# jc-bao/gym-xarm

Measured on AMD Instinct MI355X. Metric: env steps/sec (whole node), XarmPDPickAndPlace-v0, higher is better.
Workload: dtype f32

## Files before the change

### gym_xarm_amd/csrc/xarm_dev.h

```cpp
#pragma once
#include <hip/hip_runtime.h>
#include <stdio.h>
#include <stdlib.h>
#include <string.h>
#include <new>
#include "../../include/xarm_hip.h"
#include "xarm_core.h"
#include "xarm_reach_core.h"
#include "xarm_handover_core.h"
#include "xarm_handover2_core.h"
#include "xarm_stack_core.h"
#include "xarm_rearrange_core.h"
#include "xarm_coop_core.h"
#include "xarm_handover_coop_core.h"
#include "xarm_reach_coop_core.h"

namespace xd {

constexpr int WG = 64;

struct DevLds {
    float *base;
    __device__ __forceinline__ float &operator[](int i) const { return base[i * WG]; }
};

struct KParams {
    float *state;
    int64_t stride;
    int64_t num_envs;
    xk::EnvCfg cfg;
    int auto_reset;
    int state_dim;
    int coop_limit;
    int eject_coop_cap;
    xr::EnvCfg rcfg;
    xh::EnvCfg hcfg;
};

__device__ __forceinline__ int64_t late_index(int64_t e) {
    int lo = (int)e, hi = (int)(e >> 32);
    asm volatile("" : "+v"(lo), "+v"(hi) : : "memory");
    return ((int64_t)hi << 32) | (uint32_t)lo;
}

__device__ __forceinline__ void load_state(const KParams &P, int64_t e, xk::EnvState<float> &s) {
    const float *S = P.state + e;
    const int64_t n = P.stride;
#pragma unroll
    for (int i = 0; i < 9; i++) { s.q[i] = S[(xk::S_Q + i) * n]; s.qd[i] = S[(xk::S_QD + i) * n]; }
#pragma unroll
    for (int i = 0; i < 3; i++) {
        s.bp[i] = S[(xk::S_BP + i) * n]; s.bv[i] = S[(xk::S_BV + i) * n];
        s.bw[i] = S[(xk::S_BW + i) * n]; s.goal[i] = S[(xk::S_GOAL + i) * n];
    }
#pragma unroll
    for (int i = 0; i < 4; i++) s.bq[i] = S[(xk::S_BQ + i) * n];
#pragma unroll
    for (int i = 0; i < 8; i++) { s.lam_t[i] = S[(xk::S_LT + i) * n]; s.lam_p[i] = S[(xk::S_LP + i) * n]; }
    s.touch = S[xk::S_TOUCH * n]; s.mug = S[xk::S_MUG * n]; s.steps = S[xk::S_STEPS * n]; s.episode = S[xk::S_EPISODE * n];
}

__device__ __forceinline__ void store_state(const KParams &P, int64_t e, const xk::EnvState<float> &s) {
    float *S = P.state + e;
    const int64_t n = P.stride;
#pragma unroll
    for (int i = 0; i < 9; i++) { S[(xk::S_Q + i) * n] = s.q[i]; S[(xk::S_QD + i) * n] = s.qd[i]; }
#pragma unroll
    for (int i = 0; i < 3; i++) {
        S[(xk::S_BP + i) * n] = s.bp[i]; S[(xk::S_BV + i) * n] = s.bv[i];
        S[(xk::S_BW + i) * n] = s.bw[i]; S[(xk::S_GOAL + i) * n] = s.goal[i];
    }
#pragma unroll
    for (int i = 0; i < 4; i++) S[(xk::S_BQ + i) * n] = s.bq[i];
#pragma unroll
    for (int i = 0; i < 8; i++) { S[(xk::S_LT + i) * n] = s.lam_t[i]; S[(xk::S_LP + i) * n] = s.lam_p[i]; }
    S[xk::S_TOUCH * n] = s.touch; S[xk::S_MUG * n] = s.mug; S[xk::S_STEPS * n] = s.steps; S[xk::S_EPISODE * n] = s.episode;
}

__device__ __forceinline__ void write_obs(const float (&obs)[xk::OBS_DIM], const xk::EnvState<float> &s, int64_t e,
                                          float *obs_out, float *ag_out, float *dg_out) {
    float4 *o = reinterpret_cast<float4 *>(obs_out + e * xk::OBS_DIM);
#pragma unroll
    for (int k = 0; k < xk::OBS_DIM / 4; k++) o[k] = make_float4(obs[4 * k], obs[4 * k + 1], obs[4 * k + 2], obs[4 * k + 3]);
#pragma unroll
    for (int k = 0; k < 3; k++) { ag_out[e * 3 + k] = s.bp[k]; dg_out[e * 3 + k] = s.goal[k]; }
}

constexpr int FAST_LDS_FLOATS = xk::LDS_FLOATS - xk::LDS_TBL;

struct FastLds {
    float *base;
    __device__ __forceinline__ float &operator[](int i) const { return base[(i - xk::LDS_TBL) * WG]; }
};

constexpr int COOP_ENVS = WG / xc::GL;
constexpr int HO_COOP_LDS_FLOATS = xk::LDS_T;

__device__ __forceinline__ int64_t xcd_contiguous_block() {
    const unsigned b = blockIdx.x, nwg = gridDim.x, xcd = b & 7u, q = nwg >> 3, r = nwg & 7u;
    return (int64_t)((xcd < r ? xcd * (q + 1) : r * (q + 1) + (xcd - r) * q) + (b >> 3));
}

struct DppXchg {
    __device__ __forceinline__ float from0(float v) const { return __int_as_float(__builtin_amdgcn_update_dpp(0, __float_as_int(v), 0xA0, 0xF, 0xF, true)); }
    __device__ __forceinline__ float from1(float v) const { return __int_as_float(__builtin_amdgcn_update_dpp(0, __float_as_int(v), 0xF5, 0xF, 0xF, true)); }
    __device__ __forceinline__ float partner(float v) const { return __int_as_float(__builtin_amdgcn_update_dpp(0, __float_as_int(v), 0xB1, 0xF, 0xF, true)); }
};

struct HoStage {
    int tick0, tick1;
    float *qt;
    uint8_t *flag;
};
__device__ __forceinline__ void ho_load_qt(const KParams &P, const HoStage &S, int64_t e, int arm, float (&qt)[9]) {
#pragma unroll
    for (int i = 0; i < 9; i++) qt[i] = S.qt[(9 * arm + i) * P.stride + e];
}
__device__ __forceinline__ void ho_store_qt(const KParams &P, const HoStage &S, int64_t e, int arm, const float (&qt)[9]) {
#pragma unroll
    for (int i = 0; i < 9; i++) S.qt[(9 * arm + i) * P.stride + e] = qt[i];
}
__device__ __forceinline__ void ho_load(const KParams &P, int64_t e, int arm, xh::Lane<float> &L) {
    const float *S = P.state + e;
    const int64_t n = P.stride;
#pragma unroll
    for (int i = 0; i < 9; i++) { L.st.q[i] = S[(xh::H_Q + 9 * arm + i) * n]; L.st.qd[i] = S[(xh::H_QD + 9 * arm + i) * n]; }
    L.ft = S[(xh::H_FT + arm) * n];
#pragma unroll
    for (int i = 0; i < 3; i++) {
        L.st.bp[i] = S[(xh::H_BP + i) * n]; L.st.bv[i] = S[(xh::H_BV + i) * n];
        L.st.bw[i] = S[(xh::H_BW + i) * n]; L.st.goal[i] = S[(xh::H_GOAL + i) * n];
    }
#pragma unroll
    for (int i = 0; i < 4; i++) { L.st.bq[i] = S[(xh::H_BQ + i) * n]; L.st.lam_p[i] = S[(xh::H_LP + 4 * arm + i) * n]; L.st.lam_p[4 + i] = 0.f; }
#pragma unroll
    for (int i = 0; i < 8; i++) L.st.lam_t[i] = S[(xh::H_LT + i) * n];
    L.st.touch = S[(xh::H_TOUCH + arm) * n]; L.st.mug = S[(xh::H_MUG + arm) * n];
    L.st.steps = S[xh::H_STEPS * n]; L.st.episode = S[xh::H_EPISODE * n];
}

__device__ __forceinline__ void ho_store(const KParams &P, int64_t e, int arm, const xh::Lane<float> &L) {
    float *S = P.state + e;
    const int64_t n = P.stride;
#pragma unroll
    for (int i = 0; i < 9; i++) { S[(xh::H_Q + 9 * arm + i) * n] = L.st.q[i]; S[(xh::H_QD + 9 * arm + i) * n] = L.st.qd[i]; }
    S[(xh::H_FT + arm) * n] = L.ft;
#pragma unroll
    for (int i = 0; i < 4; i++) S[(xh::H_LP + 4 * arm + i) * n] = L.st.lam_p[i];
    S[(xh::H_TOUCH + arm) * n] = L.st.touch; S[(xh::H_MUG + arm) * n] = L.st.mug;
    if (arm == 0) {
#pragma unroll
        for (int i = 0; i < 3; i++) {
            S[(xh::H_BP + i) * n] = L.st.bp[i]; S[(xh::H_BV + i) * n] = L.st.bv[i];
            S[(xh::H_BW + i) * n] = L.st.bw[i]; S[(xh::H_GOAL + i) * n] = L.st.goal[i];
        }
#pragma unroll
        for (int i = 0; i < 4; i++) S[(xh::H_BQ + i) * n] = L.st.bq[i];
#pragma unroll
        for (int i = 0; i < 8; i++) S[(xh::H_LT + i) * n] = L.st.lam_t[i];
        S[xh::H_STEPS * n] = L.st.steps; S[xh::H_EPISODE * n] = L.st.episode;
    }
}

__device__ __forceinline__ void ho_write_obs(const xh::Lane<float> &L, int64_t e, int arm, float *obs_out, float *ag_out, float *dg_out) {
    float o8[8];
    xh::arm_obs(L, arm, o8);
    float *o = obs_out + e * xh::OBS_DIM;
#pragma unroll
    for (int k = 0; k < 8; k++) o[13 + 8 * arm + k] = o8[k];
    if (arm == 0) {
#pragma unroll
        for (int k = 0; k < 3; k++) { o[k] = L.st.bp[k]; o[7 + k] = L.st.bv[k]; o[10 + k] = L.st.bw[k]; ag_out[e * 3 + k] = L.st.bp[k]; dg_out[e * 3 + k] = L.st.goal[k]; }
#pragma unroll
        for (int k = 0; k < 4; k++) o[3 + k] = L.st.bq[k];
    }
}

__global__ __launch_bounds__(WG) void k_init(KParams P);
__global__ __launch_bounds__(WG) void k_step(KParams P, const float *__restrict__ actions, float *__restrict__ obs_out,
                                             float *__restrict__ ag_out, float *__restrict__ dg_out,
                                             float *__restrict__ rew_out, uint8_t *__restrict__ done_out,
                                             uint8_t *__restrict__ succ_out, float *__restrict__ term_obs,
                                             int *__restrict__ done_list, int *__restrict__ done_count,
                                             const int *__restrict__ list, const int *__restrict__ count);
__global__ __launch_bounds__(WG) void k_step_fast(KParams P, const float *__restrict__ actions, float *__restrict__ obs_out,
                                                  float *__restrict__ ag_out, float *__restrict__ dg_out,
                                                  float *__restrict__ rew_out, uint8_t *__restrict__ done_out,
                                                  uint8_t *__restrict__ succ_out, float *__restrict__ term_obs,
                                                  int *__restrict__ done_list, int *__restrict__ done_count,
                                                  int *__restrict__ eject_list, int *__restrict__ eject_count);
__global__ __launch_bounds__(WG) void k_step_lazy(KParams P, const float *__restrict__ actions, float *__restrict__ obs_out,
                                                  float *__restrict__ ag_out, float *__restrict__ dg_out,
                                                  float *__restrict__ rew_out, uint8_t *__restrict__ done_out,
                                                  uint8_t *__restrict__ succ_out);
__global__ __launch_bounds__(WG) void k_reset(KParams P, const int *__restrict__ list, const int *__restrict__ count,
                                              float *__restrict__ obs_out, float *__restrict__ ag_out,
                                              float *__restrict__ dg_out);
__global__ __launch_bounds__(WG) void k_reset_coop(KParams P, const int *__restrict__ list, const int *__restrict__ count,
                                                   float *__restrict__ obs_out, float *__restrict__ ag_out,
                                                   float *__restrict__ dg_out);
__global__ __launch_bounds__(WG) void k_step_coop(KParams P, const float *__restrict__ actions, float *__restrict__ obs_out,
                                                  float *__restrict__ ag_out, float *__restrict__ dg_out,
                                                  float *__restrict__ rew_out, uint8_t *__restrict__ done_out,
                                                  uint8_t *__restrict__ succ_out, float *__restrict__ term_obs,
                                                  int *__restrict__ done_list, int *__restrict__ done_count);
__global__ __launch_bounds__(WG) void k_step_coop_list(KParams P, const float *__restrict__ actions, float *__restrict__ obs_out,
                                                       float *__restrict__ ag_out, float *__restrict__ dg_out,
                                                       float *__restrict__ rew_out, uint8_t *__restrict__ done_out,
                                                       uint8_t *__restrict__ succ_out, float *__restrict__ term_obs,
                                                       int *__restrict__ done_list, int *__restrict__ done_count,
                                                       const int *__restrict__ list, const int *__restrict__ count);
__global__ __launch_bounds__(WG) void k_step_fast_stage(KParams P, const float *__restrict__ actions, float *__restrict__ obs_out,
                                                        float *__restrict__ ag_out, float *__restrict__ dg_out,
                                                        float *__restrict__ rew_out, uint8_t *__restrict__ done_out,
                                                        uint8_t *__restrict__ succ_out, float *__restrict__ term_obs,
                                                        int *__restrict__ done_list, int *__restrict__ done_count,
                                                        int *__restrict__ eject_list, int *__restrict__ eject_count, HoStage stage);
__global__ __launch_bounds__(WG) void k_step_from_stage(KParams P, const float *__restrict__ actions, float *__restrict__ obs_out,
                                                        float *__restrict__ ag_out, float *__restrict__ dg_out,
                                                        float *__restrict__ rew_out, uint8_t *__restrict__ done_out,
                                                        uint8_t *__restrict__ succ_out, float *__restrict__ term_obs,
                                                        int *__restrict__ done_list, int *__restrict__ done_count,
                                                        const int *__restrict__ list, const int *__restrict__ count, HoStage stage);
__global__ __launch_bounds__(WG) void k_step_coop_list_stage(KParams P, const float *__restrict__ actions, float *__restrict__ obs_out,
                                                             float *__restrict__ ag_out, float *__restrict__ dg_out,
                                                             float *__restrict__ rew_out, uint8_t *__restrict__ done_out,
                                                             uint8_t *__restrict__ succ_out, float *__restrict__ term_obs,
                                                             int *__restrict__ done_list, int *__restrict__ done_count,
                                                             const int *__restrict__ list, const int *__restrict__ count, HoStage stage);
__global__ __launch_bounds__(WG) void k_substeps(KParams P, const float *__restrict__ qt_in, int n);
__global__ void k_compact_mask(const uint8_t *__restrict__ mask, int64_t n, int *__restrict__ list, int *__restrict__ count);
__global__ void k_get_state(KParams P, float *__restrict__ out);
__global__ void k_set_state(KParams P, const float *__restrict__ in);
__global__ void k_compute_reward(int reward_type, const float *__restrict__ ag, const float *__restrict__ g, int64_t n,
                                 float *__restrict__ out);
__global__ __launch_bounds__(WG) void k_reach_init(KParams P);
__global__ __launch_bounds__(WG) void k_reach_step(KParams P, const float *__restrict__ actions, float *__restrict__ obs_out,
                                                   float *__restrict__ ag_out, float *__restrict__ dg_out,
                                                   float *__restrict__ rew_out, uint8_t *__restrict__ done_out,
                                                   uint8_t *__restrict__ succ_out, float *__restrict__ term_obs,
                                                   int *__restrict__ done_list, int *__restrict__ done_count);
__global__ __launch_bounds__(WG) void k_reach_reset(KParams P, const int *__restrict__ list, const int *__restrict__ count,
                                                    float *__restrict__ obs_out, float *__restrict__ ag_out,
                                                    float *__restrict__ dg_out);
__global__ __launch_bounds__(WG) void k_reach_step_coop(KParams P, const float *__restrict__ actions, float *__restrict__ obs_out,
                                                        float *__restrict__ ag_out, float *__restrict__ dg_out,
                                                        float *__restrict__ rew_out, uint8_t *__restrict__ done_out,
                                                        uint8_t *__restrict__ succ_out, float *__restrict__ term_obs,
                                                        int *__restrict__ done_list, int *__restrict__ done_count);
__global__ __launch_bounds__(WG) void k_reach_reset_coop(KParams P, const int *__restrict__ list, const int *__restrict__ count,
                                                         float *__restrict__ obs_out, float *__restrict__ ag_out,
                                                         float *__restrict__ dg_out);
__global__ void k_reach_compute_reward(int reward_type, const float *__restrict__ ag, const float *__restrict__ g, int64_t n,
                                       float *__restrict__ out);
__global__ __launch_bounds__(WG) void k_ho_init(KParams P);
template <typename Scene>
__global__ __launch_bounds__(WG) void k_ho_step(KParams P, const float *__restrict__ actions, float *__restrict__ obs_out,
                                                float *__restrict__ ag_out, float *__restrict__ dg_out,
                                                float *__restrict__ rew_out, uint8_t *__restrict__ done_out,
                                                uint8_t *__restrict__ succ_out, float *__restrict__ term_obs,
                                                int *__restrict__ done_list, int *__restrict__ done_count,
                                                const int *__restrict__ list, const int *__restrict__ count, HoStage stage);
template <typename Scene>
__global__ __launch_bounds__(WG) void k_ho_reset(KParams P, const int *__restrict__ list, const int *__restrict__ count,
                                                 float *__restrict__ obs_out, float *__restrict__ ag_out, float *__restrict__ dg_out);
__global__ void k_ho_compute_reward(const float *__restrict__ ag, const float *__restrict__ g, int64_t n, float *__restrict__ out);
template <typename Scene>
__global__ __launch_bounds__(WG) void k_ho_step_fast(KParams P, const float *__restrict__ actions, float *__restrict__ obs_out,
                                                     float *__restrict__ ag_out, float *__restrict__ dg_out,
                                                     float *__restrict__ rew_out, uint8_t *__restrict__ done_out,
                                                     uint8_t *__restrict__ succ_out, float *__restrict__ term_obs,
                                                     int *__restrict__ done_list, int *__restrict__ done_count,
                                                     int *__restrict__ eject_list, int *__restrict__ eject_count, HoStage stage);
template <typename Scene, bool FORCE_COUPLED>
__global__ __launch_bounds__(WG) void k_ho_step_coop_list(KParams P, const float *__restrict__ actions, float *__restrict__ obs_out,
                                                          float *__restrict__ ag_out, float *__restrict__ dg_out,
                                                          float *__restrict__ rew_out, uint8_t *__restrict__ done_out,
                                                          uint8_t *__restrict__ succ_out, float *__restrict__ term_obs,
                                                          int *__restrict__ done_list, int *__restrict__ done_count,
                                                          const int *__restrict__ list, const int *__restrict__ count, HoStage stage);
template <typename Scene, bool FORCE_COUPLED>
__global__ __launch_bounds__(WG) void k_ho_reset_coop(KParams P, const int *__restrict__ list, const int *__restrict__ count,
                                                      float *__restrict__ obs_out, float *__restrict__ ag_out, float *__restrict__ dg_out);
__global__ __launch_bounds__(WG) void k_ho2_init(KParams P);
template <typename Scene>
__global__ __launch_bounds__(WG) void k_ho2_step(KParams P, const float *__restrict__ actions, float *__restrict__ obs_out,
                                                 float *__restrict__ ag_out, float *__restrict__ dg_out,
                                                 float *__restrict__ rew_out, uint8_t *__restrict__ done_out,
                                                 uint8_t *__restrict__ succ_out, float *__restrict__ term_obs,
                                                 int *__restrict__ done_list, int *__restrict__ done_count);
template <typename Scene>
__global__ __launch_bounds__(WG) void k_ho2_reset(KParams P, const int *__restrict__ list, const int *__restrict__ count,
                                                  float *__restrict__ obs_out, float *__restrict__ ag_out, float *__restrict__ dg_out);
__global__ void k_ho2_compute_reward(const float *__restrict__ ag, const float *__restrict__ g, int64_t n, float *__restrict__ out);
__global__ __launch_bounds__(WG) void k_st_init(KParams P);
__global__ void k_class_hist(const uint8_t *__restrict__ key, int64_t n, int *__restrict__ hist);
__global__ void k_class_place(const uint8_t *__restrict__ key, int64_t n, const int *__restrict__ hist, int *__restrict__ cursor,
                              int *__restrict__ order, int group);
__global__ __launch_bounds__(WG) void k_st_step(KParams P, const float *__restrict__ actions, float *__restrict__ obs_out,
                                                float *__restrict__ ag_out, float *__restrict__ dg_out,
                                                float *__restrict__ rew_out, uint8_t *__restrict__ done_out,
                                                uint8_t *__restrict__ succ_out, float *__restrict__ term_obs,
                                                int *__restrict__ done_list, int *__restrict__ done_count,
                                                const int *__restrict__ order, uint8_t *__restrict__ key);
__global__ __launch_bounds__(WG) void k_st_reset(KParams P, const int *__restrict__ list, const int *__restrict__ count,
                                                 float *__restrict__ obs_out, float *__restrict__ ag_out, float *__restrict__ dg_out,
                                                 uint8_t *__restrict__ key);
__global__ void k_st_compute_reward(int reward_type, const float *__restrict__ ag, const float *__restrict__ g, int64_t n, float *__restrict__ out);
__global__ __launch_bounds__(WG) void k_ra_init(KParams P);
__global__ void k_ra_class_hist(const uint8_t *__restrict__ key, int64_t n, int *__restrict__ hist);
__global__ void k_ra_class_place(const uint8_t *__restrict__ key, int64_t n, const int *__restrict__ hist, int *__restrict__ cursor,
                                 int *__restrict__ order, int group);
__global__ __launch_bounds__(WG) void k_ra_step(KParams P, const float *__restrict__ actions, float *__restrict__ obs_out,
                                                float *__restrict__ ag_out, float *__restrict__ dg_out,
                                                float *__restrict__ rew_out, uint8_t *__restrict__ done_out,
                                                uint8_t *__restrict__ succ_out, float *__restrict__ term_obs,
                                                int *__restrict__ done_list, int *__restrict__ done_count,
                                                const int *__restrict__ order, uint8_t *__restrict__ key);
__global__ __launch_bounds__(WG) void k_ra_reset(KParams P, const int *__restrict__ list, const int *__restrict__ count,
                                                 float *__restrict__ obs_out, float *__restrict__ ag_out, float *__restrict__ dg_out,
                                                 uint8_t *__restrict__ key);
__global__ void k_ra_compute_reward(int reward_type, const float *__restrict__ ag, const float *__restrict__ g, int64_t n, float *__restrict__ out);
__global__ void k_episode_steps(KParams P, int steps_field, int32_t *__restrict__ out);

}
```

### gym_xarm_amd/csrc/xarm_hip.hip

```cpp
#include <stdio.h>
#include <stdlib.h>
#include <string.h>
#include <new>
#include "xarm_dev.h"
#include "xarm_render_core.h"

using namespace xd;


struct xarm_handle {
    xarm_config cfg;
    KParams kp;
    int *done_list;
    int *counters;
    int *done_count;
    int *mask_count;
    int coop_step_limit;
    int fast_pipeline;
    int *eject_list;
    int *eject_count;
    int *done_list_b;
    hipStream_t side;
    hipEvent_t ev_fork, ev_join;
    int reset_overlap;
    static constexpr int MAX_ST = XARM_HO_MAX_STAGES;
    int ho_stages;
    int ho_tick[MAX_ST + 1];
    float *ho_qt;
    uint8_t *ho_flag;
    hipStream_t st_side[MAX_ST];
    hipEvent_t st_fork[MAX_ST], st_join[MAX_ST];
    int ho_force_coupled;
    uint8_t *class_key;
    int *class_hist;
    int *class_order;
    char err[512];
    int timing;
    static constexpr int NEV = 1024;
    hipEvent_t ev0[NEV], ev1[NEV], ev2[NEV];
    int ev_n;
    double ev_ms, ev_reset_ms;
    int64_t ev_launches;
    bool ev_created;
};

static char g_err[512] = "";

static int fail(xarm_handle *h, int code, const char *fmt, const char *detail) {
    char *dst = h ? h->err : g_err;
    snprintf(dst, 512, fmt, detail);
    return code;
}
#define HIPCHK(h, call)                                                          \
    do {                                                                         \
        hipError_t _e = (call);                                                  \
        if (_e != hipSuccess) return fail(h, XARM_E_HIP, #call ": %s", hipGetErrorString(_e)); \
    } while (0)

static unsigned ho_coop_grid(int64_t cap) {
    const int64_t g = (cap + xhc::ROW_ENVS - 1) / xhc::ROW_ENVS;
    return (unsigned)(g < 1 ? 1 : (g > 2048 ? 2048 : g));
}
static void launch_ho_coop_step(xarm_handle *h, unsigned g_, const float *actions_dev, float *obs_dev, float *ag_dev, float *dg_dev, float *reward_dev,
                                uint8_t *done_dev, uint8_t *success_dev, float *terminal_obs_dev, int *done_list, int *done_count,
                                const int *list, const int *count, HoStage stage, hipStream_t st) {
    if (h->kp.hcfg.use_stand) k_ho_step_coop_list<xh::HandoverStandScene, false><<<dim3(g_), dim3(WG), 0, st>>>(
        h->kp, actions_dev, obs_dev, ag_dev, dg_dev, reward_dev, done_dev, success_dev, terminal_obs_dev, done_list, done_count, list, count, stage);
    else if (h->ho_force_coupled) k_ho_step_coop_list<xh::HandoverScene, true><<<dim3(g_), dim3(WG), 0, st>>>(
        h->kp, actions_dev, obs_dev, ag_dev, dg_dev, reward_dev, done_dev, success_dev, terminal_obs_dev, done_list, done_count, list, count, stage);
    else k_ho_step_coop_list<xh::HandoverScene, false><<<dim3(g_), dim3(WG), 0, st>>>(
        h->kp, actions_dev, obs_dev, ag_dev, dg_dev, reward_dev, done_dev, success_dev, terminal_obs_dev, done_list, done_count, list, count, stage);
}
static void launch_ho_reset(xarm_handle *h, unsigned grid2, const int *list, const int *count, float *obs_dev, float *ag_dev, float *dg_dev,
                            hipStream_t st) {
    if (h->cfg.num_obj == 2) {
        if (h->kp.hcfg.use_stand) k_ho2_reset<xh::HandoverStandScene><<<dim3(grid2), dim3(WG), 0, st>>>(h->kp, list, count, obs_dev, ag_dev, dg_dev);
        else k_ho2_reset<xh::HandoverScene><<<dim3(grid2), dim3(WG), 0, st>>>(h->kp, list, count, obs_dev, ag_dev, dg_dev);
        return;
    }
    const int64_t cap = h->kp.num_envs < (int64_t)h->kp.coop_limit ? h->kp.num_envs : (int64_t)h->kp.coop_limit;
    if (cap > 0) {
        if (h->kp.hcfg.use_stand) k_ho_reset_coop<xh::HandoverStandScene, false><<<dim3(ho_coop_grid(cap)), dim3(WG), 0, st>>>(h->kp, list, count, obs_dev, ag_dev, dg_dev);
        else if (h->ho_force_coupled) k_ho_reset_coop<xh::HandoverScene, true><<<dim3(ho_coop_grid(cap)), dim3(WG), 0, st>>>(h->kp, list, count, obs_dev, ag_dev, dg_dev);
        else k_ho_reset_coop<xh::HandoverScene, false><<<dim3(ho_coop_grid(cap)), dim3(WG), 0, st>>>(h->kp, list, count, obs_dev, ag_dev, dg_dev);
    }
    if (h->kp.num_envs > cap) {
        if (h->kp.hcfg.use_stand) k_ho_reset<xh::HandoverStandScene><<<dim3(grid2), dim3(WG), 0, st>>>(h->kp, list, count, obs_dev, ag_dev, dg_dev);
        else k_ho_reset<xh::HandoverScene><<<dim3(grid2), dim3(WG), 0, st>>>(h->kp, list, count, obs_dev, ag_dev, dg_dev);
    }
}

static void launch_reach_reset(xarm_handle *h, const int *list, const int *count, float *obs_dev, float *ag_dev, float *dg_dev, hipStream_t st) {
    const int64_t cap = h->kp.num_envs < (int64_t)h->kp.coop_limit ? h->kp.num_envs : (int64_t)h->kp.coop_limit;
    if (cap > 0)
        k_reach_reset_coop<<<dim3((unsigned)((cap + COOP_ENVS - 1) / COOP_ENVS)), dim3(WG), 0, st>>>(h->kp, list, count, obs_dev, ag_dev, dg_dev);
    if (h->kp.num_envs > cap)
        k_reach_reset<<<dim3((unsigned)(h->kp.stride / WG)), dim3(WG), 0, st>>>(h->kp, list, count, obs_dev, ag_dev, dg_dev);
}

static void launch_pnp_reset(xarm_handle *h, const int *list, const int *count, float *obs_dev, float *ag_dev, float *dg_dev,
                             hipStream_t st) {
    const int64_t cap = h->kp.num_envs < (int64_t)h->kp.coop_limit ? h->kp.num_envs : (int64_t)h->kp.coop_limit;
    if (cap > 0)
        k_reset_coop<<<dim3((unsigned)((cap + COOP_ENVS - 1) / COOP_ENVS)), dim3(WG), 0, st>>>(h->kp, list, count, obs_dev, ag_dev, dg_dev);
    if (h->kp.num_envs > cap)
        k_reset<<<dim3((unsigned)(h->kp.stride / WG)), dim3(WG), 0, st>>>(h->kp, list, count, obs_dev, ag_dev, dg_dev);
}

struct DeviceGuard {
    int prev;
    bool switched;
    explicit DeviceGuard(int dev) : prev(-1), switched(false) {
        if (hipGetDevice(&prev) == hipSuccess && prev != dev) switched = hipSetDevice(dev) == hipSuccess;
    }
    ~DeviceGuard() { if (switched) hipSetDevice(prev); }
};
#define DEVGUARD(h) DeviceGuard _guard((h)->cfg.device)

static void timing_flush(xarm_handle *h) {
    for (int i = 0; i < h->ev_n; i++) {
        float ms = 0.f;
        if (hipEventSynchronize(h->ev2[i]) == hipSuccess && hipEventElapsedTime(&ms, h->ev0[i], h->ev1[i]) == hipSuccess) {
            h->ev_ms += ms;
            h->ev_launches++;
            if (hipEventElapsedTime(&ms, h->ev1[i], h->ev2[i]) == hipSuccess) h->ev_reset_ms += ms;
        }
    }
    h->ev_n = 0;
}

extern "C" {

#define XARM_STR2(x) #x
#define XARM_STR(x) XARM_STR2(x)
#ifdef XARM_SWEEP_VARIANT
const char *xarm_version(void) { return "xarm_hip 0.1 (gfx950) TIMING VARIANT sweeps=" XARM_STR(XARM_SWEEP_VARIANT); }
#else
const char *xarm_version(void) { return "xarm_hip 0.1 (gfx950)"; }
#endif

const char *xarm_last_error(const xarm_handle *h) { return h ? h->err : g_err; }

int xarm_create(const xarm_config *cfg, xarm_handle **out) {
    if (!cfg || !out) return fail(nullptr, XARM_E_INVALID, "%s", "xarm_create: null argument");
    const bool reach = cfg->env_kind == XARM_ENV_REACH, handover = cfg->env_kind == XARM_ENV_HANDOVER, stack = cfg->env_kind == XARM_ENV_STACK_TOWER;
    const bool rearrange = cfg->env_kind == XARM_ENV_REARRANGE;
    if (cfg->env_kind != XARM_ENV_PICK_AND_PLACE && !reach && !handover && !stack && !rearrange) return fail(nullptr, XARM_E_INVALID, "%s", "xarm_create: unsupported env_kind");
    if (stack && cfg->num_obj != 3) return fail(nullptr, XARM_E_INVALID, "%s", "xarm_create: XarmStackTower has num_obj == 3 (xarm_stack_tower.py:19)");
    if (stack && cfg->reward_type > 1) return fail(nullptr, XARM_E_INVALID, "%s", "xarm_create: XarmStackTower reward_type is 0 (sparse) or 1 (-d)");
    if (rearrange && cfg->num_obj != 4) return fail(nullptr, XARM_E_INVALID, "%s", "xarm_create: XarmRearrange has num_obj == 4 (xarm_rearrange.py:20)");
    if (rearrange && cfg->reward_type > 1) return fail(nullptr, XARM_E_INVALID, "%s", "xarm_create: XarmRearrange reward_type is 0 (sparse) or 1 (-d)");
    if (handover && cfg->num_obj != 1 && cfg->num_obj != 2) return fail(nullptr, XARM_E_INVALID, "%s", "xarm_create: XarmHandover supports num_obj 1 or 2");
    if (handover && cfg->num_obj == 2 && cfg->reward_type != 0)
        return fail(nullptr, XARM_E_INVALID, "%s", "xarm_create: XarmHandover with num_obj == 2 takes the sparse reward (the reference's dense branch raises a broadcast error there, xarm_handover.py:187-188)");
    if (!reach && !stack && !rearrange && !handover && cfg->num_obj != 1)
        return fail(nullptr, XARM_E_INVALID, "%s", "xarm_create: XarmPickAndPlace supports num_obj == 1 (with more the reference's own step raises, xarm_pick_and_place.py:289-291)");
    if (handover && cfg->reward_type != 0 && cfg->reward_type != XARM_REWARD_DENSE)
        return fail(nullptr, XARM_E_INVALID, "%s", "xarm_create: XarmHandover reward_type is sparse (hard-wired in the reference, xarm_handover.py:40) or dense (:184-199)");
    if (cfg->use_stand && !handover) return fail(nullptr, XARM_E_INVALID, "%s", "xarm_create: use_stand belongs to XarmHandover (xarm_handover.py:391-392)");
    if (cfg->auto_reset < 0 || cfg->auto_reset > XARM_AUTO_RESET_LAZY) return fail(nullptr, XARM_E_INVALID, "%s", "xarm_create: auto_reset must be 0, 1 or XARM_AUTO_RESET_LAZY");
    if (cfg->auto_reset == XARM_AUTO_RESET_LAZY && cfg->env_kind != XARM_ENV_PICK_AND_PLACE)
        return fail(nullptr, XARM_E_INVALID, "%s", "xarm_create: lazy auto-reset is implemented for XarmPickAndPlace only");
    if (cfg->num_envs <= 0 || cfg->num_envs > (int64_t)1 << 30) return fail(nullptr, XARM_E_INVALID, "%s", "xarm_create: num_envs out of range");
    if (cfg->reward_type < 0 || cfg->reward_type > 2) return fail(nullptr, XARM_E_INVALID, "%s", "xarm_create: unsupported reward_type");
    if (!reach && !stack && !rearrange && cfg->goal_shape != XARM_GOAL_AIR && cfg->goal_shape != XARM_GOAL_GROUND)
        return fail(nullptr, XARM_E_INVALID, "%s", "xarm_create: unsupported goal_shape");
    int ndev = 0;
    if (hipGetDeviceCount(&ndev) != hipSuccess || ndev <= 0) return fail(nullptr, XARM_E_NODEVICE, "%s", "xarm_create: no HIP device");
    if (cfg->device < 0 || cfg->device >= ndev) return fail(nullptr, XARM_E_INVALID, "%s", "xarm_create: bad device ordinal");
    DeviceGuard _guard(cfg->device);
    xarm_handle *h = new (std::nothrow) xarm_handle();
    if (!h) return fail(nullptr, XARM_E_INVALID, "%s", "xarm_create: out of host memory");
    memset(h, 0, sizeof *h);
    h->cfg = *cfg;
    const int64_t E = cfg->num_envs, stride = (E + WG - 1) / WG * WG;
    h->kp.stride = stride;
    h->kp.num_envs = E;
    h->kp.cfg.seed = cfg->seed;
    h->kp.cfg.env_id_offset = cfg->env_id_offset;
    h->kp.cfg.init_grasp_rate = cfg->init_grasp_rate;
    h->kp.cfg.goal_ground_rate = cfg->goal_ground_rate;
    h->kp.cfg.goal_shape = cfg->goal_shape;
    h->kp.cfg.reward_type = cfg->reward_type;
    h->kp.auto_reset = cfg->auto_reset;
    h->kp.coop_limit = 0;
    if (cfg->env_kind == XARM_ENV_PICK_AND_PLACE || cfg->env_kind == XARM_ENV_REACH) {
        h->kp.coop_limit = cfg->reset_coop_limit > 0 ? cfg->reset_coop_limit : (cfg->reset_coop_limit < 0 ? 0 : XARM_RESET_COOP_LIMIT_DEFAULT);
        const char *ev = getenv("XARM_RESET_COOP_LIMIT");
        if (ev && *ev && cfg->reset_coop_limit == 0) h->kp.coop_limit = atoi(ev) > 0 ? atoi(ev) : 0;
    }
    h->coop_step_limit = (cfg->env_kind != XARM_ENV_PICK_AND_PLACE && cfg->env_kind != XARM_ENV_REACH) || cfg->step_coop_limit < 0 ? 0 :
                         (cfg->step_coop_limit > 0 ? cfg->step_coop_limit : XARM_STEP_COOP_LIMIT_DEFAULT);
    {
        const char *ev = getenv("XARM_STEP_COOP_LIMIT");
        if (ev && *ev && cfg->step_coop_limit == 0 && (cfg->env_kind == XARM_ENV_PICK_AND_PLACE || cfg->env_kind == XARM_ENV_REACH))
            h->coop_step_limit = atoi(ev) > 0 ? atoi(ev) : 0;
    }
    const bool handover2 = handover && cfg->num_obj == 2;
    const bool handover1 = handover && !handover2;
    if (handover1 && cfg->step_coop_limit >= 0) {
        h->coop_step_limit = cfg->step_coop_limit > 0 ? cfg->step_coop_limit : XARM_HO_STEP_COOP_LIMIT_DEFAULT;
        const char *ev = getenv("XARM_STEP_COOP_LIMIT");
        if (ev && *ev && cfg->step_coop_limit == 0) h->coop_step_limit = atoi(ev) > 0 ? atoi(ev) : 0;
    }
    if (handover1) {
        h->kp.coop_limit = cfg->reset_coop_limit > 0 ? cfg->reset_coop_limit : (cfg->reset_coop_limit < 0 ? 0 : XARM_HO_RESET_COOP_LIMIT_DEFAULT);
        const char *ev = getenv("XARM_RESET_COOP_LIMIT");
        if (ev && *ev && cfg->reset_coop_limit == 0) h->kp.coop_limit = atoi(ev) > 0 ? atoi(ev) : 0;
    }
    h->fast_pipeline = ((cfg->env_kind == XARM_ENV_PICK_AND_PLACE || handover1) && cfg->step_coop_limit >= 0 && cfg->auto_reset != XARM_AUTO_RESET_LAZY) ? 1 : 0;
    {
        const char *ev = getenv("XARM_STEP_PIPELINE");
        if (ev && *ev) h->fast_pipeline = h->fast_pipeline && atoi(ev) != 0;
        ev = getenv("XARM_HO_FORCE_COUPLED");
        h->ho_force_coupled = ev && *ev && atoi(ev) != 0;
        h->ho_stages = handover1 && h->fast_pipeline ? XARM_HO_STAGES_DEFAULT : 1;
        ev = getenv("XARM_HO_STAGES");
        if (ev && *ev && handover1 && h->fast_pipeline) h->ho_stages = atoi(ev) < 1 ? 1 : (atoi(ev) > xarm_handle::MAX_ST ? xarm_handle::MAX_ST : atoi(ev));
        const bool pnp_pipe = cfg->env_kind == XARM_ENV_PICK_AND_PLACE && h->fast_pipeline;
        if (pnp_pipe) h->ho_stages = XARM_PNP_STAGES_DEFAULT;
        ev = getenv("XARM_PNP_STAGES");
        if (ev && *ev && pnp_pipe) h->ho_stages = atoi(ev) < 1 ? 1 : (atoi(ev) > xarm_handle::MAX_ST ? xarm_handle::MAX_ST : atoi(ev));
        static_assert(xm::HO_N_TICKS == xm::PNP_N_SUBSTEPS, "one stage table for both");
        for (int c = 0; c <= h->ho_stages; c++) h->ho_tick[c] = c * xm::HO_N_TICKS / h->ho_stages;
        ev = getenv("XARM_HO_STAGE_TICKS");
        if (ev && *ev && h->ho_stages > 1) {
            int c = 1, prev = 0;
            const char *q = ev;
            while (*q && c < h->ho_stages) {
                const int v = atoi(q);
                if (v <= prev || v >= xm::HO_N_TICKS) break;
                h->ho_tick[c++] = prev = v;
                while (*q && *q != ',') q++;
                if (*q == ',') q++;
            }
            if (c != h->ho_stages) for (int k = 0; k <= h->ho_stages; k++) h->ho_tick[k] = k * xm::HO_N_TICKS / h->ho_stages;
        }
    }
    h->kp.eject_coop_cap = handover1 ? XARM_HO_EJECT_COOP_CAP : XARM_EJECT_COOP_CAP;
    if (cfg->step_coop_limit == 1) h->kp.eject_coop_cap = 0x7fffffff;
    h->kp.state_dim = reach ? xr::STATE_DIM : (handover2 ? xh2::STATE_DIM : (handover ? xh::STATE_DIM : (stack ? xs::STATE_DIM : (rearrange ? xra::STATE_DIM : xk::STATE_DIM))));
    h->kp.hcfg.seed = cfg->seed;
    h->kp.hcfg.env_id_offset = cfg->env_id_offset;
    h->kp.hcfg.same_side_rate = cfg->same_side_rate;
    h->kp.hcfg.goal_shape = cfg->goal_shape;
    h->kp.hcfg.use_stand = handover && cfg->use_stand ? 1 : 0;
    h->kp.hcfg.reward_type = cfg->reward_type == XARM_REWARD_DENSE ? 1 : 0;
    h->kp.rcfg.seed = cfg->seed;
    h->kp.rcfg.env_id_offset = cfg->env_id_offset;
    h->kp.rcfg.reward_type = cfg->reward_type;
    hipError_t e1 = hipMalloc(&h->kp.state, sizeof(float) * h->kp.state_dim * stride);
    hipError_t e2 = hipMalloc(&h->done_list, sizeof(int) * stride);
    static_assert(xra::NCLS >= xs::NCLS, "one counter block serves both class orders");
    hipError_t e3 = hipMalloc(&h->counters, sizeof(int) * (3 + 2 * xra::NCLS));
    h->done_count = h->counters; h->eject_count = h->counters + 1; h->class_hist = h->counters + 3;
    hipError_t e4 = hipMalloc(&h->mask_count, sizeof(int));
    if (e4 == hipSuccess && h->fast_pipeline) {
        e4 = hipMalloc(&h->eject_list, sizeof(int) * stride * h->ho_stages);
        if (e4 == hipSuccess) e4 = hipMalloc(&h->done_list_b, sizeof(int) * stride);
        const char *ev = getenv("XARM_RESET_OVERLAP");
        if (e4 == hipSuccess && cfg->auto_reset && !handover1 && !(ev && *ev && atoi(ev) == 0)) {
            e4 = hipStreamCreateWithFlags(&h->side, hipStreamNonBlocking);
            if (e4 == hipSuccess) e4 = hipEventCreateWithFlags(&h->ev_fork, hipEventDisableTiming);
            if (e4 == hipSuccess) e4 = hipEventCreateWithFlags(&h->ev_join, hipEventDisableTiming);
            h->reset_overlap = e4 == hipSuccess;
        }
    }
    if (e4 == hipSuccess && h->fast_pipeline && h->ho_stages > 1) {
        e4 = hipMalloc(&h->ho_qt, sizeof(float) * 18 * stride);
        if (e4 == hipSuccess) e4 = hipMalloc(&h->ho_flag, stride);
        if (e4 == hipSuccess) e4 = hipMemset(h->ho_flag, 0, stride);
        for (int c = 0; c + 1 < h->ho_stages && e4 == hipSuccess; c++) {
            const char *pv = getenv("XARM_HO_SIDE_PRIO");
            int lo = 0, hi = 0;
            hipDeviceGetStreamPriorityRange(&lo, &hi);
            if (pv && *pv && atoi(pv) != 0) e4 = hipStreamCreateWithPriority(&h->st_side[c], hipStreamNonBlocking, lo);
            else e4 = hipStreamCreateWithFlags(&h->st_side[c], hipStreamNonBlocking);
            if (e4 == hipSuccess) e4 = hipEventCreateWithFlags(&h->st_fork[c], hipEventDisableTiming);
            if (e4 == hipSuccess) e4 = hipEventCreateWithFlags(&h->st_join[c], hipEventDisableTiming);
        }
    }
    if (e4 == hipSuccess && (stack || rearrange)) {
        const char *ev = getenv(stack ? "XARM_ST_CLASS_ORDER" : "XARM_RA_CLASS_ORDER");
        if (!(ev && *ev && atoi(ev) == 0)) {
            e4 = hipMalloc(&h->class_key, stride);
            if (e4 == hipSuccess) e4 = hipMalloc(&h->class_order, sizeof(int) * stride);
            if (e4 == hipSuccess) e4 = hipMemset(h->class_key, 0, stride);
        }
    }
    if (e1 != hipSuccess || e2 != hipSuccess || e3 != hipSuccess || e4 != hipSuccess) {
        fail(nullptr, XARM_E_HIP, "xarm_create: hipMalloc failed: %s", hipGetErrorString(e1 != hipSuccess ? e1 : (e2 != hipSuccess ? e2 : (e3 != hipSuccess ? e3 : e4))));
        xarm_destroy(h);
        return XARM_E_HIP;
    }
    hipMemset(h->kp.state, 0, sizeof(float) * h->kp.state_dim * stride);
    hipMemset(h->counters, 0, sizeof(int) * (3 + 2 * xra::NCLS));
    hipMemset(h->mask_count, 0, sizeof(int));
    if (reach) k_reach_init<<<dim3((unsigned)(stride / WG)), dim3(WG)>>>(h->kp);
    else if (handover2) k_ho2_init<<<dim3((unsigned)(2 * stride / WG)), dim3(WG)>>>(h->kp);
    else if (handover) k_ho_init<<<dim3((unsigned)(2 * stride / WG)), dim3(WG)>>>(h->kp);
    else if (stack) k_st_init<<<dim3((unsigned)(2 * stride / WG)), dim3(WG)>>>(h->kp);
    else if (rearrange) k_ra_init<<<dim3((unsigned)(2 * stride / WG)), dim3(WG)>>>(h->kp);
    else k_init<<<dim3((unsigned)(stride / WG)), dim3(WG)>>>(h->kp);
    hipError_t e5 = hipDeviceSynchronize();
    if (e5 != hipSuccess) {
        fail(nullptr, XARM_E_HIP, "xarm_create: k_init: %s", hipGetErrorString(e5));
        xarm_destroy(h);
        return XARM_E_HIP;
    }
    *out = h;
    return XARM_OK;
}

int xarm_destroy(xarm_handle *h) {
    if (!h) return XARM_OK;
    DEVGUARD(h);
    hipDeviceSynchronize();
    if (h->ev_created)
        for (int i = 0; i < xarm_handle::NEV; i++) { hipEventDestroy(h->ev0[i]); hipEventDestroy(h->ev1[i]); hipEventDestroy(h->ev2[i]); }
    if (h->kp.state) hipFree(h->kp.state);
    if (h->done_list) hipFree(h->done_list);
    if (h->counters) hipFree(h->counters);
    if (h->mask_count) hipFree(h->mask_count);
    if (h->eject_list) hipFree(h->eject_list);
    if (h->done_list_b) hipFree(h->done_list_b);
    if (h->ev_fork) hipEventDestroy(h->ev_fork);
    if (h->ev_join) hipEventDestroy(h->ev_join);
    if (h->side) hipStreamDestroy(h->side);
    if (h->class_key) hipFree(h->class_key);
    if (h->class_order) hipFree(h->class_order);
    if (h->ho_qt) hipFree(h->ho_qt);
    if (h->ho_flag) hipFree(h->ho_flag);
    for (int c = 0; c < xarm_handle::MAX_ST; c++) {
        if (h->st_fork[c]) hipEventDestroy(h->st_fork[c]);
        if (h->st_join[c]) hipEventDestroy(h->st_join[c]);
        if (h->st_side[c]) hipStreamDestroy(h->st_side[c]);
    }
    delete h;
    return XARM_OK;
}

int xarm_dims(const xarm_handle *h, xarm_dims_t *out) {
    if (!out) return XARM_E_INVALID;
// ... 390 lines not shown
```

### gym_xarm_amd/csrc/xarm_k_pnp_coop.hip

```cpp
#include "xarm_dev.h"

namespace xd {

__global__ __launch_bounds__(WG) void k_reset_coop(KParams P, const int *__restrict__ list, const int *__restrict__ count,
                                                   float *__restrict__ obs_out, float *__restrict__ ag_out,
                                                   float *__restrict__ dg_out) {
    __shared__ float smem[xk::LDS_FLOATS * WG];
    const int64_t n = count ? (int64_t)*count : P.num_envs;
    if (n > P.coop_limit) return;
    const int64_t i0 = (list ? (int64_t)blockIdx.x : xcd_contiguous_block()) * COOP_ENVS;
    if (i0 >= n) return;
    const int64_t i_raw = i0 + threadIdx.x / xc::GL;
    const bool live = i_raw < n;
    const int64_t i = live ? i_raw : n - 1;
    const int64_t e_in = list ? (int64_t)list[i] : i;
    const xc::Grp G{(int)(threadIdx.x & (xc::GL - 1))};
    DevLds lds{smem + threadIdx.x};
    xk::EnvState<float> s;
    load_state(P, e_in, s);
    xc::env_reset<float, DevLds>(G, P.cfg, e_in, s, lds);
    if (!live || G.l != 0) return;
    const int64_t e = late_index(e_in);
    store_state(P, e, s);
    if (obs_out) {
        float obs[xk::OBS_DIM];
        xk::get_obs(s, obs);
        write_obs(obs, s, e, obs_out, ag_out, dg_out);
    }
}

__global__ __launch_bounds__(WG) void k_step_coop(KParams P, const float *__restrict__ actions, float *__restrict__ obs_out,
                                                  float *__restrict__ ag_out, float *__restrict__ dg_out,
                                                  float *__restrict__ rew_out, uint8_t *__restrict__ done_out,
                                                  uint8_t *__restrict__ succ_out, float *__restrict__ term_obs,
                                                  int *__restrict__ done_list, int *__restrict__ done_count) {
    __shared__ float smem[xk::LDS_FLOATS * WG];
    const int64_t e_raw = xcd_contiguous_block() * COOP_ENVS + threadIdx.x / xc::GL;
    const bool live = e_raw < P.num_envs;
    const int64_t e_in = live ? e_raw : P.num_envs - 1;
    const xc::Grp G{(int)(threadIdx.x & (xc::GL - 1))};
    DevLds lds{smem + threadIdx.x};
    xk::EnvState<float> s;
    load_state(P, e_in, s);
    const float4 a4 = reinterpret_cast<const float4 *>(actions)[e_in];
    const float act[4] = {a4.x, a4.y, a4.z, a4.w};
    float obs[xk::OBS_DIM], reward;
    bool done, success;
    xc::env_step<float, DevLds>(G, P.cfg, s, act, obs, reward, done, success, lds);
    if (!live || G.l != 0) return;
    const int64_t e = late_index(e_in);
    store_state(P, e, s);
    write_obs(obs, s, e, obs_out, ag_out, dg_out);
    rew_out[e] = reward;
    done_out[e] = done ? 1 : 0;
    succ_out[e] = success ? 1 : 0;
    if (done && P.auto_reset) {
        if (term_obs) {
            float4 *o = reinterpret_cast<float4 *>(term_obs + e * xk::OBS_DIM);
#pragma unroll
            for (int k = 0; k < xk::OBS_DIM / 4; k++) o[k] = make_float4(obs[4 * k], obs[4 * k + 1], obs[4 * k + 2], obs[4 * k + 3]);
        }
        const int pos = atomicAdd(done_count, 1);
        done_list[pos] = (int)e;
    }
}

__global__ __launch_bounds__(WG) void k_step_coop_list(KParams P, const float *__restrict__ actions, float *__restrict__ obs_out,
                                                       float *__restrict__ ag_out, float *__restrict__ dg_out,
                                                       float *__restrict__ rew_out, uint8_t *__restrict__ done_out,
                                                       uint8_t *__restrict__ succ_out, float *__restrict__ term_obs,
                                                       int *__restrict__ done_list, int *__restrict__ done_count,
                                                       const int *__restrict__ list, const int *__restrict__ count) {
    __shared__ float smem[xk::LDS_FLOATS * WG];
    const int64_t n = (int64_t)*count;
    if (n > P.eject_coop_cap) return;
    const xc::Grp G{(int)(threadIdx.x & (xc::GL - 1))};
    DevLds lds{smem + threadIdx.x};
#pragma unroll 1
    for (int64_t i0 = (int64_t)blockIdx.x * COOP_ENVS; i0 < n; i0 += (int64_t)gridDim.x * COOP_ENVS) {
        const int64_t i_raw = i0 + threadIdx.x / xc::GL;
        const bool live = i_raw < n;
        const int64_t e_in = (int64_t)list[live ? i_raw : n - 1];
        xk::EnvState<float> s;
        load_state(P, e_in, s);
        const float4 a4 = reinterpret_cast<const float4 *>(actions)[e_in];
        const float act[4] = {a4.x, a4.y, a4.z, a4.w};
        float obs[xk::OBS_DIM], reward;
        bool done, success;
        xc::env_step<float, DevLds>(G, P.cfg, s, act, obs, reward, done, success, lds);
        if (live && G.l == 0) {
            const int64_t e = late_index(e_in);
            store_state(P, e, s);
            write_obs(obs, s, e, obs_out, ag_out, dg_out);
            rew_out[e] = reward;
            done_out[e] = done ? 1 : 0;
            succ_out[e] = success ? 1 : 0;
            if (done && P.auto_reset) {
                if (term_obs) {
                    float4 *o = reinterpret_cast<float4 *>(term_obs + e * xk::OBS_DIM);
#pragma unroll
                    for (int k = 0; k < xk::OBS_DIM / 4; k++) o[k] = make_float4(obs[4 * k], obs[4 * k + 1], obs[4 * k + 2], obs[4 * k + 3]);
                }
                const int pos = atomicAdd(done_count, 1);
                done_list[pos] = (int)e;
            }
        }
    }
}

__global__ __launch_bounds__(WG) void k_step_coop_list_stage(KParams P, const float *__restrict__ actions, float *__restrict__ obs_out,
                                                             float *__restrict__ ag_out, float *__restrict__ dg_out,
                                                             float *__restrict__ rew_out, uint8_t *__restrict__ done_out,
                                                             uint8_t *__restrict__ succ_out, float *__restrict__ term_obs,
                                                             int *__restrict__ done_list, int *__restrict__ done_count,
                                                             const int *__restrict__ list, const int *__restrict__ count, HoStage stage) {
    __shared__ float smem[xk::LDS_FLOATS * WG];
    const int64_t n = (int64_t)*count;
    if (n > P.eject_coop_cap) return;
    const xc::Grp G{(int)(threadIdx.x & (xc::GL - 1))};
    DevLds lds{smem + threadIdx.x};
#pragma unroll 1
    for (int64_t i0 = (int64_t)blockIdx.x * COOP_ENVS; i0 < n; i0 += (int64_t)gridDim.x * COOP_ENVS) {
        const int64_t i_raw = i0 + threadIdx.x / xc::GL;
        const bool live = i_raw < n;
        const int64_t e_in = (int64_t)list[live ? i_raw : n - 1];
        xk::EnvState<float> s;
        load_state(P, e_in, s);
        const float4 a4 = reinterpret_cast<const float4 *>(actions)[e_in];
        const float act[4] = {a4.x, a4.y, a4.z, a4.w};
        float obs[xk::OBS_DIM], reward, qt[9];
        bool done, success;
        if (stage.tick0 > 0) ho_load_qt(P, stage, e_in, 0, qt);
        xc::env_step_from<float, DevLds>(G, P.cfg, s, act, qt, stage.tick0, obs, reward, done, success, lds);
        if (live && G.l == 0) {
            const int64_t e = late_index(e_in);
            store_state(P, e, s);
            write_obs(obs, s, e, obs_out, ag_out, dg_out);
            rew_out[e] = reward;
            done_out[e] = done ? 1 : 0;
            succ_out[e] = success ? 1 : 0;
            if (done && P.auto_reset) {
                if (term_obs) {
                    float4 *o = reinterpret_cast<float4 *>(term_obs + e * xk::OBS_DIM);
#pragma unroll
                    for (int k = 0; k < xk::OBS_DIM / 4; k++) o[k] = make_float4(obs[4 * k], obs[4 * k + 1], obs[4 * k + 2], obs[4 * k + 3]);
                }
                const int pos = atomicAdd(done_count, 1);
                done_list[pos] = (int)e;
            }
        }
    }
}

}
```

Measured before the change: 15.94 million.

## Spread small cooperative reset batches across more waves to fill idle CUs

When the reset list is small, the cooperative reset kernel now gives each wave only one or two environments instead of the full COOP_ENVS, and the host widens the grid up to four waves per CU. This spreads a few resetting envs across more compute units so the reset pass has less serial latency. The cost is redundant lanes: rows beyond the per-wave count compute duplicate work that is masked out. It also adds a device attribute query and an env override, XARM_RESET_LANES.

```diff
diff --git a/gym_xarm_amd/csrc/xarm_dev.h b/gym_xarm_amd/csrc/xarm_dev.h
--- a/gym_xarm_amd/csrc/xarm_dev.h
+++ b/gym_xarm_amd/csrc/xarm_dev.h
@@ -94,6 +94,15 @@
 };
 
 constexpr int COOP_ENVS = WG / xc::GL;
+struct CoopWidth {
+    int wave_slots;
+    int min_epw;
+};
+__device__ __forceinline__ int coop_envs_per_wave(int64_t n, CoopWidth w) {
+    if (w.min_epw <= 1 && n <= (int64_t)w.wave_slots) return 1;
+    if (w.min_epw <= 2 && n <= 2 * (int64_t)w.wave_slots) return 2;
+    return COOP_ENVS;
+}
 constexpr int HO_COOP_LDS_FLOATS = xk::LDS_T;
 
 __device__ __forceinline__ int64_t xcd_contiguous_block() {
@@ -198,7 +207,7 @@
                                               float *__restrict__ dg_out);
 __global__ __launch_bounds__(WG) void k_reset_coop(KParams P, const int *__restrict__ list, const int *__restrict__ count,
                                                    float *__restrict__ obs_out, float *__restrict__ ag_out,
-                                                   float *__restrict__ dg_out);
+                                                   float *__restrict__ dg_out, CoopWidth width);
 __global__ __launch_bounds__(WG) void k_step_coop(KParams P, const float *__restrict__ actions, float *__restrict__ obs_out,
                                                   float *__restrict__ ag_out, float *__restrict__ dg_out,
                                                   float *__restrict__ rew_out, uint8_t *__restrict__ done_out,
diff --git a/gym_xarm_amd/csrc/xarm_hip.hip b/gym_xarm_amd/csrc/xarm_hip.hip
--- a/gym_xarm_amd/csrc/xarm_hip.hip
+++ b/gym_xarm_amd/csrc/xarm_hip.hip
@@ -2,6 +2,7 @@
 #include <stdlib.h>
 #include <string.h>
 #include <new>
+#include <algorithm>
 #include "xarm_dev.h"
 #include "xarm_render_core.h"
 
@@ -23,6 +24,7 @@
     hipStream_t side;
     hipEvent_t ev_fork, ev_join;
     int reset_overlap;
+    CoopWidth reset_width;
     static constexpr int MAX_ST = XARM_HO_MAX_STAGES;
     int ho_stages;
     int ho_tick[MAX_ST + 1];
@@ -101,8 +103,15 @@
 static void launch_pnp_reset(xarm_handle *h, const int *list, const int *count, float *obs_dev, float *ag_dev, float *dg_dev,
                              hipStream_t st) {
     const int64_t cap = h->kp.num_envs < (int64_t)h->kp.coop_limit ? h->kp.num_envs : (int64_t)h->kp.coop_limit;
-    if (cap > 0)
-        k_reset_coop<<<dim3((unsigned)((cap + COOP_ENVS - 1) / COOP_ENVS)), dim3(WG), 0, st>>>(h->kp, list, count, obs_dev, ag_dev, dg_dev);
+    if (cap > 0) {
+        int64_t grid = (cap + COOP_ENVS - 1) / COOP_ENVS;
+        const CoopWidth w = h->reset_width;
+        if (list && w.wave_slots > 0 && w.min_epw < COOP_ENVS) {
+            const int64_t wide = std::min<int64_t>((cap + w.min_epw - 1) / w.min_epw, w.wave_slots);
+            grid = std::max(grid, wide);
+        }
+        k_reset_coop<<<dim3((unsigned)grid), dim3(WG), 0, st>>>(h->kp, list, count, obs_dev, ag_dev, dg_dev, w);
+    }
     if (h->kp.num_envs > cap)
         k_reset<<<dim3((unsigned)(h->kp.stride / WG)), dim3(WG), 0, st>>>(h->kp, list, count, obs_dev, ag_dev, dg_dev);
 }
@@ -189,6 +198,14 @@
         const char *ev = getenv("XARM_RESET_COOP_LIMIT");
         if (ev && *ev && cfg->reset_coop_limit == 0) h->kp.coop_limit = atoi(ev) > 0 ? atoi(ev) : 0;
     }
+    {
+        int cus = 0;
+        if (hipDeviceGetAttribute(&cus, hipDeviceAttributeMultiprocessorCount, cfg->device) != hipSuccess) cus = 0;
+        h->reset_width.wave_slots = 4 * cus;
+        h->reset_width.min_epw = 1;
+        const char *ev = getenv("XARM_RESET_LANES");
+        if (ev && *ev) h->reset_width.min_epw = atoi(ev) >= 64 ? 1 : (atoi(ev) >= 32 ? 2 : COOP_ENVS);
+    }
     h->coop_step_limit = (cfg->env_kind != XARM_ENV_PICK_AND_PLACE && cfg->env_kind != XARM_ENV_REACH) || cfg->step_coop_limit < 0 ? 0 :
                          (cfg->step_coop_limit > 0 ? cfg->step_coop_limit : XARM_STEP_COOP_LIMIT_DEFAULT);
     {
diff --git a/gym_xarm_amd/csrc/xarm_k_pnp_coop.hip b/gym_xarm_amd/csrc/xarm_k_pnp_coop.hip
--- a/gym_xarm_amd/csrc/xarm_k_pnp_coop.hip
+++ b/gym_xarm_amd/csrc/xarm_k_pnp_coop.hip
@@ -4,15 +4,17 @@
 
 __global__ __launch_bounds__(WG) void k_reset_coop(KParams P, const int *__restrict__ list, const int *__restrict__ count,
                                                    float *__restrict__ obs_out, float *__restrict__ ag_out,
-                                                   float *__restrict__ dg_out) {
+                                                   float *__restrict__ dg_out, CoopWidth width) {
     __shared__ float smem[xk::LDS_FLOATS * WG];
     const int64_t n = count ? (int64_t)*count : P.num_envs;
     if (n > P.coop_limit) return;
-    const int64_t i0 = (list ? (int64_t)blockIdx.x : xcd_contiguous_block()) * COOP_ENVS;
+    const int epw = list ? coop_envs_per_wave(n, width) : COOP_ENVS;
+    const int row = (int)(threadIdx.x / xc::GL);
+    const int64_t i0 = (list ? (int64_t)blockIdx.x : xcd_contiguous_block()) * epw;
     if (i0 >= n) return;
-    const int64_t i_raw = i0 + threadIdx.x / xc::GL;
-    const bool live = i_raw < n;
-    const int64_t i = live ? i_raw : n - 1;
+    const int64_t i_raw = i0 + (row & (epw - 1));
+    const int64_t i = i_raw < n ? i_raw : n - 1;
+    const bool live = i_raw < n && row < epw;
     const int64_t e_in = list ? (int64_t)list[i] : i;
     const xc::Grp G{(int)(threadIdx.x & (xc::GL - 1))};
     DevLds lds{smem + threadIdx.x};
```

After: 16.12 million (median of 6 runs). 1.1% higher.
